# ZHANGKEON/DIS-YOLO

Hardware: AMD Instinct MI355X
Metric: train images/sec @576x576 bf16 (higher is better)
Workload: dtype bf16

## Files before the change

### dis-yolo_amd/csrc/bn.hip

```cpp
#include <stdio.h>
#include <stdlib.h>
#include "common.h"
#include "runtime.h"

namespace {

constexpr int FIN_CPB = 4;
template <int Q>
__device__ __forceinline__ bool block_sum_partials(const float* part, int rows, int C, double* res , int* c_out) {
  constexpr int LANES = 256 / FIN_CPB;
  __shared__ double sh[LANES][FIN_CPB][Q];
  const int cl = threadIdx.x % FIN_CPB, g = threadIdx.x / FIN_CPB;
  const int c = blockIdx.x * FIN_CPB + cl;
  double acc[Q];
#pragma unroll
  for (int q = 0; q < Q; ++q) acc[q] = 0.0;
  if (c < C) {
    int r = g;
    for (; r + 3 * LANES < rows; r += 4 * LANES) {
      float v[4][Q];
#pragma unroll
      for (int u = 0; u < 4; ++u)
#pragma unroll
        for (int q = 0; q < Q; ++q) v[u][q] = part[((size_t)(r + u * LANES) * C + c) * Q + q];
// ... 372 lines not shown
  return ((size_t)colreduce_blocks(rows, C) * C * 2 + 2 * (size_t)C) * sizeof(float);
}

extern "C" int disyolo_bn_act_bwd(const void* dy, const void* x, const float* scale, const float* shift,
                                  const float* mean, const float* rstd, void* dx, float* dgamma, float* dbeta,
                                  int64_t rows, int C, float alpha, void* shortcut_grad, int shortcut_accumulate,
                                  void* workspace, size_t workspace_bytes, void* stream) {
  DY_REQUIRE(dy && x && scale && shift && mean && rstd && dx && dgamma && dbeta, "bn_act_bwd: null pointer");
  DY_REQUIRE(rows > 0 && C > 0 && C % 8 == 0, "bn_act_bwd: bad shape");
  if (workspace_bytes < disyolo_bn_act_bwd_workspace(rows, C) || !workspace) {
    disyolo_set_error("bn_act_bwd: workspace too small");
    return DISYOLO_E_WORKSPACE;
  }
  DY_RECORD_OR_RUN([=](void* s) { return disyolo_bn_act_bwd(dy, x, scale, shift, mean, rstd, dx, dgamma, dbeta, rows, C, alpha, shortcut_grad, shortcut_accumulate, workspace, workspace_bytes, s); });
  hipStream_t s = (hipStream_t)stream;
  const int nb = colreduce_blocks(rows, C), rpb = colreduce_rpb(rows, C);
  const int chunks = C / 8, cpb = chunks < 256 ? chunks : 256;
  float* part = (float*)workspace;
  float* c1 = part + (size_t)nb * C * 2;
  float* c2 = c1 + C;
  hipLaunchKernelGGL(colreduce_kernel<1>, dim3(nb, ceil_div(chunks, cpb)), dim3(256), 0, s, (const uint4*)dy,
                     (const uint4*)x, scale, shift, mean, rstd, alpha, rows, C, rpb, part);
  DY_CHECK_LAUNCH();
  hipLaunchKernelGGL(bn_bwd_finalize_kernel, dim3(ceil_div(C, FIN_CPB)), dim3(256), 0, s, part, nb, C, 1.0 / (double)rows,
                     scale, mean, rstd, dgamma, dbeta, c1, c2);
  DY_CHECK_LAUNCH();
  const int64_t nvec = rows * C / 8;
  hipLaunchKernelGGL(bn_bwd_apply_kernel, dim3(grid_for(nvec)), dim3(256), 0, s, (const uint4*)dy, (const uint4*)x,
                     scale, shift, c1, c2, (uint4*)dx, nvec, C, alpha, (uint4*)shortcut_grad, shortcut_accumulate);
  DY_CHECK_LAUNCH();
  return DISYOLO_OK;
}

extern "C" size_t disyolo_bn_act_bwd_partials_workspace(int C) { return C > 0 ? 2 * (size_t)C * sizeof(float) : 0; }

extern "C" int disyolo_bn_act_bwd_partials(const void* dy, const void* x, const float* scale, const float* shift,
                                           const float* mean, const float* rstd, void* dx, float* dgamma, float* dbeta,
                                           int64_t rows, int C, float alpha, const float* partials, int part_rows,
                                           void* shortcut_grad, int shortcut_accumulate, void* workspace,
                                           size_t workspace_bytes, void* stream) {
  DY_REQUIRE(dy && x && scale && shift && mean && rstd && dx && dgamma && dbeta && partials, "bn_act_bwd_partials: null pointer");
  DY_REQUIRE(rows > 0 && C > 0 && C % 8 == 0 && part_rows > 0, "bn_act_bwd_partials: bad shape");
  if (workspace_bytes < disyolo_bn_act_bwd_partials_workspace(C) || !workspace) {
    disyolo_set_error("bn_act_bwd_partials: workspace too small");
    return DISYOLO_E_WORKSPACE;
  }
  DY_RECORD_OR_RUN([=](void* s) {
    return disyolo_bn_act_bwd_partials(dy, x, scale, shift, mean, rstd, dx, dgamma, dbeta, rows, C, alpha, partials, part_rows,
                                       shortcut_grad, shortcut_accumulate, workspace, workspace_bytes, s);
  });
  hipStream_t s = (hipStream_t)stream;
  float* c1 = (float*)workspace;
  float* c2 = c1 + C;
  hipLaunchKernelGGL(bn_bwd_finalize_kernel, dim3(ceil_div(C, FIN_CPB)), dim3(256), 0, s, partials, part_rows, C,
                     1.0 / (double)rows, scale, mean, rstd, dgamma, dbeta, c1, c2);
  DY_CHECK_LAUNCH();
  const int64_t nvec = rows * C / 8;
  hipLaunchKernelGGL(bn_bwd_apply_kernel, dim3(grid_for(nvec)), dim3(256), 0, s, (const uint4*)dy, (const uint4*)x,
                     scale, shift, c1, c2, (uint4*)dx, nvec, C, alpha, (uint4*)shortcut_grad, shortcut_accumulate);
  DY_CHECK_LAUNCH();
  return DISYOLO_OK;
}

extern "C" int disyolo_bn_partial_sums(const float* partials, int rows, int C, double* sums, void* stream) {
  DY_REQUIRE(partials && sums && rows > 0 && C > 0, "bn_partial_sums: bad args");
  DY_RECORD_OR_RUN([=](void* s) { return disyolo_bn_partial_sums(partials, rows, C, sums, s); });
// ... 122 lines not shown
```

### dis-yolo_amd/lib.py

```python
from __future__ import annotations

import ctypes as C
import os
from typing import Optional

import numpy as np
import torch

_HERE = os.path.dirname(os.path.abspath(__file__))
LIB_PATH = os.environ.get("DISYOLO_LIB", os.path.join(_HERE, "libdisyolo_hip.so"))

GRAD_LD = 32
ROI_MAX = 16
ROI_W = 12
K_MAPS = (3, 5, 7)
MASK_STRIDES = (1, 2, 4)


def roi_w(k: int) -> int:
    return 2 * (k + 1) + 4


def block32_post(k: int) -> int:
    return {3: 1, 5: 2, 7: 3}[k]
# ... 58 lines not shown
    "disyolo_conv_first_fwd_fp8": (C.c_int, [C.c_void_p] * 5 + [C.c_float] + [C.c_int] * 4 + [C.c_float, C.c_void_p]),
    "disyolo_quant_fp8": (C.c_int, [C.c_void_p, C.c_int, C.c_void_p, C.c_int64, C.c_float, C.c_void_p]),
    "disyolo_dequant_fp8": (C.c_int, [C.c_void_p, C.c_void_p, C.c_int64, C.c_float, C.c_void_p]),
    "disyolo_pack_weights_fp8": (C.c_int, [C.c_void_p, C.c_void_p] + [C.c_int] * 3 + [C.c_float, C.c_void_p]),
    "disyolo_conv2d_wgrad_plan": (C.c_int, [C.POINTER(ConvDesc), C.c_int] + [C.POINTER(C.c_int)] * 4),
    "disyolo_conv_first_wgrad_workspace": (C.c_size_t, [C.c_int] * 4),
    "disyolo_conv_first_wgrad": (C.c_int, [C.c_void_p] * 3 + [C.c_int] * 4 + [C.c_void_p, C.c_size_t, C.c_void_p]),
    "disyolo_image_pad8": (C.c_int, [C.c_void_p, C.c_void_p, C.c_int64, C.c_void_p]),
    "disyolo_copy2d_f32": (C.c_int, [C.c_void_p, C.c_void_p] + [C.c_int] * 4 + [C.c_void_p]),
    "disyolo_pack_weights": (C.c_int, [C.c_void_p] * 3 + [C.c_int] * 4 + [C.c_void_p]),
    "disyolo_pack_table_bytes": (C.c_size_t, [C.c_int]),
    "disyolo_pack_table_build": (C.c_int, [C.c_void_p, C.c_int, C.c_void_p, C.POINTER(C.c_int)]),
    "disyolo_pack_all": (C.c_int, [C.c_void_p, C.c_int, C.c_int, C.c_void_p]),
    "disyolo_bn_finalize": (C.c_int, [C.c_void_p, C.c_int, C.c_int, C.c_int64] + [C.c_void_p] * 4 +
                            [C.c_float, C.c_float] + [C.c_void_p] * 5),
    "disyolo_colstats_rows": (C.c_int, [C.c_int64, C.c_int]),
    "disyolo_colstats": (C.c_int, [C.c_void_p, C.c_void_p, C.c_int64, C.c_int, C.c_void_p]),
    "disyolo_bn_fold": (C.c_int, [C.c_void_p] * 4 + [C.c_float] + [C.c_void_p] * 2 + [C.c_int, C.c_void_p]),
    "disyolo_bn_act_fwd": (C.c_int, [C.c_void_p] * 5 + [C.c_int64, C.c_int, C.c_float, C.c_void_p]),
    "disyolo_bn_act_bwd_workspace": (C.c_size_t, [C.c_int64, C.c_int]),
    "disyolo_bn_act_bwd_partials_workspace": (C.c_size_t, [C.c_int]),
    "disyolo_bn_act_bwd_partials": (C.c_int, [C.c_void_p] * 9 + [C.c_int64, C.c_int, C.c_float, C.c_void_p, C.c_int,
                                              C.c_void_p, C.c_int, C.c_void_p, C.c_size_t, C.c_void_p]),
    "disyolo_bn_partial_sums": (C.c_int, [C.c_void_p, C.c_int, C.c_int, C.c_void_p, C.c_void_p]),
    "disyolo_bn_finalize_sums": (C.c_int, [C.c_void_p, C.c_int, C.c_int64] + [C.c_void_p] * 4 + [C.c_float, C.c_float] +
                                 [C.c_void_p] * 5),
    "disyolo_bn_bwd_reduce_rows": (C.c_int, [C.c_int64, C.c_int]),
    "disyolo_bn_bwd_reduce": (C.c_int, [C.c_void_p] * 6 + [C.c_int64, C.c_int, C.c_float, C.c_void_p, C.c_void_p, C.c_size_t,
                                        C.c_void_p]),
    "disyolo_bn_bwd_apply_sums": (C.c_int, [C.c_void_p] * 8 + [C.c_int64] + [C.c_void_p] * 3 + [C.c_int64, C.c_int, C.c_float,
                                            C.c_void_p, C.c_int, C.c_void_p, C.c_size_t, C.c_void_p]),
    "disyolo_bn_act_bwd": (C.c_int, [C.c_void_p] * 9 + [C.c_int64, C.c_int, C.c_float, C.c_void_p, C.c_int, C.c_void_p, C.c_size_t,
                                                       C.c_void_p]),
    "disyolo_upsample2x_bwd": (C.c_int, [C.c_void_p] * 2 + [C.c_int] * 7 + [C.c_void_p]),
    "disyolo_colsum_workspace": (C.c_size_t, [C.c_int64, C.c_int]),
    "disyolo_colsum": (C.c_int, [C.c_void_p, C.c_void_p, C.c_int64, C.c_int, C.c_int, C.c_void_p, C.c_size_t,
                                 C.c_void_p]),
    "disyolo_detect_workspace": (C.c_size_t, [C.c_int] * 3),
    "disyolo_detect": (C.c_int, [C.c_void_p] * 3 + [C.c_int] * 3 + [C.c_void_p] * 2 + [C.c_float, C.c_float, C.c_int] +
                       [C.c_void_p] * 3 + [C.c_size_t, C.c_void_p]),
    "disyolo_yolo_loss_workspace": (C.c_size_t, [C.c_int] * 3),
    "disyolo_yolo_loss": (C.c_int, [C.c_void_p, C.c_void_p, C.c_void_p] + [C.c_int] * 4 + [C.c_void_p, C.c_float] +
                          [C.c_void_p] * 4 + [C.c_size_t, C.c_void_p]),
    "disyolo_shuffle_perm": (C.c_int, [C.c_void_p, C.c_int, C.c_void_p, C.c_int, C.c_int, C.c_uint32, C.c_void_p, C.c_void_p]),
    "disyolo_mask_rois": (C.c_int, [C.c_void_p, C.c_int, C.c_void_p, C.c_int, C.c_void_p, C.c_void_p] + [C.c_int] * 4 +
                          [C.c_float, C.c_void_p, C.c_void_p, C.c_void_p]),
    "disyolo_mask_rois_k": (C.c_int, [C.c_void_p, C.c_int, C.c_void_p, C.c_int, C.c_void_p, C.c_void_p] + [C.c_int] * 5 +
                            [C.c_float, C.c_void_p, C.c_void_p, C.c_void_p]),
    "disyolo_psroi_loss_workspace": (C.c_size_t, [C.c_int, C.c_int]),
    "disyolo_psroi_loss": (C.c_int, [C.c_void_p, C.c_void_p, C.c_int, C.c_void_p, C.c_void_p] + [C.c_int] * 3 +
                           [C.c_float] + [C.c_void_p] * 3 + [C.c_size_t, C.c_void_p]),
    "disyolo_psroi_loss_s": (C.c_int, [C.c_void_p, C.c_void_p, C.c_int, C.c_void_p, C.c_void_p] + [C.c_int] * 4 +
                             [C.c_float] + [C.c_void_p] * 3 + [C.c_size_t, C.c_void_p]),
    "disyolo_psroi_assemble": (C.c_int, [C.c_void_p, C.c_void_p] + [C.c_int] * 4 + [C.c_void_p] * 3),
    "disyolo_mask_paste": (C.c_int, [C.c_void_p, C.c_int, C.c_int, C.c_void_p, C.c_void_p, C.c_int, C.c_int, C.c_void_p,
                                     C.c_void_p, C.c_void_p]),
    "disyolo_letterbox": (C.c_int, [C.c_void_p, C.c_int, C.c_int, C.c_void_p, C.c_int, C.c_void_p, C.c_void_p]),
    "disyolo_confusion16": (C.c_int, [C.c_void_p, C.c_void_p, C.c_int64, C.c_void_p, C.c_void_p]),
    "disyolo_paste_job_size": (C.c_size_t, []),
    "disyolo_paste_job_plan": (C.c_int, [C.c_void_p, C.c_int]),
    "disyolo_mask_paste_iou_batch": (C.c_int, [C.c_void_p, C.c_void_p, C.c_int, C.c_int, C.c_void_p, C.c_void_p]),
    "disyolo_adam_step": (C.c_int, [C.c_void_p] * 4 + [C.c_int64, C.c_int64] + [C.c_float] * 5 + [C.c_int64, C.c_float,
                                                                                             C.c_void_p]),
    "disyolo_adam_step_dev": (C.c_int, [C.c_void_p] * 4 + [C.c_int64, C.c_int64] + [C.c_float] * 5 + [C.c_void_p, C.c_float,
                                                                                                 C.c_void_p]),
    "disyolo_adam_fused_workspace": (C.c_size_t, [C.c_int64]),
# ... 637 lines not shown
    buf = ws.get(load().disyolo_bn_bwd_reduce_rows(rows, C_) * C_ * 2 * 4)
    _check(load().disyolo_bn_bwd_reduce(_p(dy), _p(x), _p(scale), _p(shift), _p(mean), _p(rstd), rows, C_, alpha, _p(sums),
                                        _p(buf), buf.numel(), _stream()), "bn_bwd_reduce")


def bn_bwd_apply_sums(dy, x, scale, shift, mean, rstd, local_sums, global_sums, count, dx, dgamma, dbeta, rows, C_,
                      ws: Workspace, alpha=0.1, shortcut_grad=None, shortcut_accumulate=False) -> None:
    buf = ws.get(2 * C_ * 4)
    _check(load().disyolo_bn_bwd_apply_sums(_p(dy), _p(x), _p(scale), _p(shift), _p(mean), _p(rstd), _p(local_sums),
                                            _p(global_sums), count, _p(dx), _p(dgamma), _p(dbeta), rows, C_, alpha,
                                            _p(shortcut_grad), int(shortcut_accumulate), _p(buf), buf.numel(), _stream()),
           "bn_bwd_apply_sums")


def bn_fold(gamma, beta, mm, mv, eps, scale, shift) -> None:
    _check(load().disyolo_bn_fold(_p(gamma), _p(beta), _p(mm), _p(mv), eps, _p(scale), _p(shift), gamma.numel(),
                                  _stream()), "bn_fold")


def bn_act_fwd(x, scale, shift, residual, y, rows, C_, alpha=0.1) -> None:
    _check(load().disyolo_bn_act_fwd(_p(x), _p(scale), _p(shift), _p(residual), _p(y), rows, C_, alpha, _stream()),
           "bn_act_fwd")


def bn_act_bwd(dy, x, scale, shift, mean, rstd, dx, dgamma, dbeta, rows, C_, ws: Workspace, alpha=0.1,
               shortcut_grad=None, shortcut_accumulate=False) -> None:
    need = load().disyolo_bn_act_bwd_workspace(rows, C_)
    buf = ws.get(need)
    _check(load().disyolo_bn_act_bwd(_p(dy), _p(x), _p(scale), _p(shift), _p(mean), _p(rstd), _p(dx), _p(dgamma),
                                     _p(dbeta), rows, C_, alpha, _p(shortcut_grad), int(shortcut_accumulate), _p(buf),
                                     buf.numel(), _stream()), "bn_act_bwd")


def mask_paste(masks, rects, classids, image_h: int, image_w: int, full_masks, merged) -> None:
    n = int(rects.shape[0])
    if n:
        _need(masks, torch.float32, "masks")
        _need(rects, torch.int32, "rects")
        _need(classids, torch.int32, "classids")
    _check(load().disyolo_mask_paste(_p(masks) if n else None, n, int(masks.shape[-1]) if n else 1, _p(rects) if n else None,
                                     _p(classids) if n else None, image_h, image_w, _p(full_masks), _p(merged), _stream()),
           "mask_paste")


PASTE_JOB = np.dtype([("masks", np.uint64), ("rects", np.uint64), ("classids", np.uint64), ("gt", np.uint64), ("gt_class", np.uint64),
                      ("merged", np.uint64), ("true_map", np.uint64), ("counts", np.uint64), ("n", np.int32), ("ng", np.int32),
                      ("image_h", np.int32), ("image_w", np.int32), ("block0", np.int32), ("reserved", np.int32)])
assert PASTE_JOB.itemsize == 88


def paste_job_plan(jobs) -> int:
    if jobs.dtype != PASTE_JOB or not jobs.flags["C_CONTIGUOUS"] or jobs.ndim != 1:
        raise DisyoloError("paste_job_plan: jobs must be a contiguous 1-d array of PASTE_JOB records")
    rc = load().disyolo_paste_job_plan(jobs.ctypes.data, int(jobs.shape[0]))
    if rc < 0:
        _check(rc, "paste_job_plan")
    return rc


def mask_paste_iou_batch(jobs, jobs_dev, size: int, conf=None) -> None:
    if jobs.dtype != PASTE_JOB or not jobs.flags["C_CONTIGUOUS"] or jobs.ndim != 1:
        raise DisyoloError("mask_paste_iou_batch: jobs must be a contiguous 1-d array of PASTE_JOB records")
    _need(jobs_dev, torch.uint8, "jobs_dev")
    if jobs_dev.numel() < jobs.nbytes:
        raise DisyoloError("mask_paste_iou_batch: %d jobs do not fit %d bytes" % (jobs.shape[0], jobs_dev.numel()))
    if conf is not None:
# ... 308 lines not shown
```

### dis-yolo_amd/net.py

```python
from __future__ import annotations

from typing import Dict, List, Optional, Sequence, Tuple

import math
import json
import contextlib
import os
import sys
import numpy as np
import torch

from . import config as cfg
from . import lib as L

BF16 = torch.bfloat16
F32 = torch.float32

WGRAD_GROUP = 3
OPT_CHUNK_ELEMS = 8_000_000
PIPE_LANE = 2


class Layer:
    __slots__ = ("idx", "cin", "cout", "k", "stride", "kind", "src", "src_up", "shortcut", "lock", "H", "W", "Ho",
                 "Wo", "w", "bias", "gamma", "beta", "mm", "mv", "scale", "shift", "mean", "rstd", "wp", "wdg", "raw",
                 "act", "stats", "stats_rows", "desc", "grad", "grad_set", "need_grad", "dw", "dbias", "dgamma",
                 "dbeta", "dx", "pad_t", "pad_l", "dgrad_descs", "wgrad_desc", "cout_pad",
                 "act8", "w8", "s_w", "s_out", "escale", "desc8", "dual16", "bn_sums", "bwd_local", "bwd_global", "bwd_part", "bwd_part_rows", "wq",
                 "csync", "fused_fwd", "csync_bwd", "fused_bwd")

    def __init__(self, idx, cin, cout, k, stride, kind, src, src_up=None, shortcut=None):
        self.idx, self.cin, self.cout, self.k, self.stride, self.kind = idx, cin, cout, k, stride, kind
        self.src, self.src_up, self.shortcut = src, src_up, shortcut
        for s in self.__slots__[9:]:
            setattr(self, s, None)


MASK_STRIDES = (4, 2, 1)


def build_topology(num_class: int, k_map: int, mask_stride: int = 2) -> List[Layer]:
    if mask_stride not in MASK_STRIDES:
        raise ValueError("mask_stride must be one of %s (got %r)" % (", ".join(map(str, MASK_STRIDES)), mask_stride))
    out_depth = (num_class + 5) * 3
    Ls: List[Layer] = []

    def add(idx, cin, cout, k, s, kind, src, src_up=None, shortcut=None):
        Ls.append(Layer(idx, cin, cout, k, s, kind, src, src_up, shortcut))

    add(1, 3, 32, 3, 1, "bn", 0)
    add(2, 32, 64, 3, 2, "bn", 1)
    i = 3
    ch = 64
    for nblocks, down in ((1, 5), (2, 10), (8, 27), (8, 44), (4, None)):
        for _ in range(nblocks):
            add(i, ch, ch // 2, 1, 1, "bn", i - 1)
            add(i + 1, ch // 2, ch, 3, 1, "res", i, shortcut=i - 1)
            i += 2
        if down:
            add(down, ch, ch * 2, 3, 2, "bn", down - 1)
            ch *= 2
            i = down + 1
# ... 88 lines not shown
        self.plan_only = bool(plan_only)
        if device is None:
            if self.plan_only:
                device = torch.device("cpu")
            elif not torch.cuda.is_available():
                raise L.DisyoloError("YOLONet needs a GPU: the HIP kernels have no CPU fallback")
            else:
                device = torch.device("cuda", torch.cuda.current_device())
        self.device = torch.device(device)
        if not self.plan_only:
            L.load()
            self.ws = L.Workspace(self.device)
            self.ws_aux = L.Workspace(self.device)
            self.ws_det = L.Workspace(self.device)
        self._reg_fresh = False
        self.lock = dict(lock) if lock is not None else {i: (stage == 1 and i <= 52) for i in range(1, self.score_layer + 1)}
        self.layers = build_topology(self.num_class, self.k, self.mask_stride)
        self.by_idx = {l.idx: l for l in self.layers}
        self._lr = float(cfg.LEARNING_RATE)
        self.lr_dev = None
        self.dp = None
        self.sync_bn = False
        self._rec = None
        self._prog = None
        self._prog_marks = []
        self._graph = None
        self.opt_chunks = None
        self._overlap = False
        self._overlap_rec = False
        self._tail_open = False
        self._progs = None
        self.fuse_first_two = True
        self.fuse_blocks = True
        self.use_side_lane = os.environ.get("DISYOLO_SIDE_LANE", "1") != "0"
        self.bn_inkernel = os.environ.get("DISYOLO_BN_INKERNEL", "1") != "0"
        self.bn_inkernel_bwd = os.environ.get("DISYOLO_BN_INKERNEL_BWD", "0") == "1"
        self.bn_fuse_check = None
        self.tail_on_main = 0
        self.pair = bool(backbone_pair)
        self._half = 0
        self._pair_P = 0
        self._init_params(seed, xavier_locked)
        if self.pair:
            if not self.training or self.dtype != "bf16" or self.plan_only:
                raise L.DisyoloError("backbone_pair needs a bf16 training net")
            self._pair_P = self._backbone_prefix()
            if self._pair_P < 2:
                raise L.DisyoloError("backbone_pair needs a locked layer prefix (stage 1)")
        if not self.plan_only:
            self._plan(self.batchsize, self.image_size)

    def _init_params(self, seed: int, xavier_locked: bool) -> None:
        dev = self.device
        g = torch.Generator().manual_seed(seed)
        n_decay = 0
        n_nodecay = 0
        for l in self.layers:
            l.lock = self.lock[l.idx]
            if not l.lock:
                n_decay += l.k * l.k * l.cin * l.cout + (l.cout if l.kind == "lin" else 0)
                if l.kind != "lin":
                    n_nodecay += 2 * l.cout
        self.n_decay, self.n_params = n_decay, n_decay + n_nodecay
        n = max(self.n_params, 1)
        self.arena = torch.zeros(n, dtype=F32, device=dev)
        self.grad_arena = torch.zeros(n, dtype=F32, device=dev)
# ... 922 lines not shown
            if tgt.csync_bwd is None:
                tgt.csync_bwd = L.cluster_sync_buffer(tgt.cout, self.device)
            d = L.make_conv_desc(dx, desc_kw["w"], tgt.dx, k, 1, in_div=in_div, pads=desc_kw["pads"], out_hw=desc_kw["out_hw"],
                                 residual=res, tile=tile_f,
                                 bn_bwd=(tgt.raw, tgt.scale, tgt.shift, tgt.mean, tgt.rstd, tgt.bwd_part, cfg.ALPHA),
                                 bn_bwd_fused=dict(dgamma=tgt.dgamma, dbeta=tgt.dbeta, sync=tgt.csync_bwd))
            tgt.fused_bwd = True
        L.conv2d_fwd(d)

    def check_cluster_sync(self) -> None:
        for l in self.layers:
            for name, buf in (("forward", l.csync), ("backward", l.csync_bwd)):
                if buf is not None:
                    code = L.cluster_sync_error(buf, l.cout)
                    if code:
                        raise L.DisyoloError("conv%d: the in-launch batch-norm exchange (%s) timed out (code %#x): another launch of "
                                             "that kind was running on this device, or the grid was not resident; the results of "
                                             "this run are wrong (DISYOLO_BN_INKERNEL=0 switches the feature off)" % (l.idx, name, code))

    def _shortcut_feeds_grad(self, tgt: Layer) -> bool:
        return tgt.shortcut is not None and self.by_idx[tgt.shortcut].grad is not None

    def _final_writers(self, visit) -> Dict[int, Tuple[int, str]]:
        last: Dict[int, Tuple[int, str]] = {}
        for l in visit:
            if l.lock:
                continue
            if l.kind != "lin" and l.shortcut is not None and self.by_idx[l.shortcut].grad is not None:
                last[l.shortcut] = (l.idx, "add")
            for mode, tgt, _ in l.dgrad_descs:
                last[tgt.idx] = (l.idx, mode)
        return last

    def backward_order(self) -> List[Layer]:
        heads = [self.by_idx[i] for i in (75, 74, 67, 66, 59, 58)]
        return heads + [l for l in reversed(self.layers) if l.idx not in self.HEAD_LAYERS]

    def backward(self, on_layer_done=None, sweep: bool = False) -> None:
        B = self.B
        for l in self.layers:
            l.grad_set = False
        visit = self.backward_order()
        order = [l for l in visit if not l.lock]
        final_of = {} if self.sync_bn else self._final_writers(visit)
        for l in self.layers:
            l.bwd_part_rows = 0
            l.fused_bwd = False
        inl = self.dp is not None and self.dp.inlist
        overlap_opt = sweep and (self.dp is None or inl) and self.n_params > 0
        if overlap_opt:
            if self.opt_chunks is None:
                self._plan_opt_chunks()
            self._opt_swept = set()
            self._opt_done = [set() for _ in self.opt_chunks]
        pending: list = []

        def flush():
            if not pending:
                return
            side_g = pending[0][4]
            mark = L.lane_mark(0) if side_g else None
            waited = False
            for (pl, pdx, pld, pM, pside) in pending:
                if pside:
                    if not waited:
                        L.lane_wait(mark, 1)
                        waited = True
                    L.set_lane(1)
                wsl = self.ws_aux if pside else self.ws
                if pl.kind == "lin":
                    L.colsum(pl.dx, pl.dbias, pM, pl.cout_pad, pl.cout, wsl)
                if pl.idx == 1:
                    L.conv_first_wgrad(self.images, pl.dx, pl.dw, wsl)
                else:
                    L.conv2d_wgrad(pl.wgrad_desc, pdx, pld, pl.dw, wsl)
                if pside:
                    L.set_lane(0)
                if self._overlap_rec:
                    for src, reader in self._xstep_reader.items():
                        if reader == pl.idx and self._xstep_slot[src] in self._xstep_waits.values():
                            L.lane_mark_slot(1 if pside else 0, self._xstep_slot[src])
                if overlap_opt and pside:
                    ci = self._opt_chunk_of[pl.idx]
                    self._opt_done[ci].add(pl.idx)
                    if self._opt_done[ci] == self.opt_chunks[ci]["members"]:
                        if inl:
                            L.lane_wait(L.lane_mark(1), L.COMM_LANE)
                            L.set_lane(L.COMM_LANE)
                            ch = self.opt_chunks[ci]
                            self.dp.exchange_inlist(ci, ch["off"], ch["cnt"])
                            self._sweep_chunk(ci, 1.0 / self.dp.world_size)
                            L.set_lane(0)
                        else:
                            L.set_lane(1)
                            self._sweep_chunk(ci, 1.0)
                            L.set_lane(0)
                if on_layer_done is not None:
                    on_layer_done(pl)
            pending.clear()

        for l in visit:
            pos = order.index(l) if not l.lock else -1
            if l.idx == self.score_layer and getattr(self, "_mask_loss_pending", False):
                L.lane_wait(self._mask_mark, 0)
                self._mask_loss_pending = False
            if l.lock:
                continue
            M = B * l.Ho * l.Wo
            if l.kind == "lin":
                dx, ld = l.dx, l.cout_pad
            else:
                if not l.grad_set:
                    raise L.DisyoloError("layer %d received no gradient" % l.idx)
                sc = self.by_idx[l.shortcut] if l.shortcut is not None else None
                if sc is not None and sc.grad is None:
                    sc = None
                kw = dict(shortcut_grad=sc.grad, shortcut_accumulate=sc.grad_set) if sc is not None else {}
                if l.fused_bwd:
                    pass
                elif self.sync_bn:
                    L.bn_bwd_reduce(l.grad, l.raw, l.scale, l.shift, l.mean, l.rstd, M, l.cout, l.bwd_local, self.ws, cfg.ALPHA)
                    L.copy2d_f32(l.bwd_local.view(torch.float32), l.bwd_global.view(torch.float32), 1, 4 * l.cout,
                                 4 * l.cout, 4 * l.cout)
                    self._sync_sums(l.bwd_global)
                    L.bn_bwd_apply_sums(l.grad, l.raw, l.scale, l.shift, l.mean, l.rstd, l.bwd_local, l.bwd_global,
                                        M * self.dp.world_size, l.dx, l.dgamma, l.dbeta, M, l.cout, self.ws, cfg.ALPHA, **kw)
                elif l.bwd_part_rows:
                    ref = None
                    if self.bn_fuse_check is not None and self._rec is None:
                        ref = (torch.empty_like(l.dx), torch.empty_like(l.dgamma), torch.empty_like(l.dbeta))
                        L.bn_act_bwd(l.grad, l.raw, l.scale, l.shift, l.mean, l.rstd, ref[0], ref[1], ref[2], M, l.cout,
                                     self.ws, cfg.ALPHA)
                    L.bn_act_bwd_partials(l.grad, l.raw, l.scale, l.shift, l.mean, l.rstd, l.dx, l.dgamma, l.dbeta, M,
                                          l.cout, l.bwd_part, l.bwd_part_rows, self.ws, cfg.ALPHA, **kw)
                    if ref is not None:
                        torch.cuda.synchronize()

                        def rel(a, b):
                            a, b = a.double().flatten(), b.double().flatten()
                            return float((a - b).norm() / (b.norm() + 1e-30))
                        self.bn_fuse_check.append({"layer": l.idx, "rows": l.bwd_part_rows, "shape": (l.Ho, l.Wo, l.cout),
                                                   "dx": rel(l.dx, ref[0]), "dgamma": rel(l.dgamma, ref[1]),
                                                   "dbeta": rel(l.dbeta, ref[2]),
                                                   "finite": bool(torch.isfinite(l.dx.float()).all())})
                else:
                    L.bn_act_bwd(l.grad, l.raw, l.scale, l.shift, l.mean, l.rstd, l.dx, l.dgamma, l.dbeta, M, l.cout,
                                 self.ws, cfg.ALPHA, **kw)
                dx, ld = l.dx, l.cout
                if sc is not None:
                    sc.grad_set = True
            tail = self.tail_on_main if (self.dp is None or inl) else 0
            side = self.use_side_lane and (pos < len(order) - tail)
            for mode, tgt, kw in l.dgrad_descs:
                if mode == "direct":
                    final = (final_of.get(tgt.idx) == (l.idx, "direct") and not tgt.lock and tgt.kind != "lin"
                             and tgt.cout % 8 == 0 and tgt.raw is not None)
                    self._accumulate_into(tgt, kw, dx, l.cin, l.k, l.stride, final)
                    tgt.grad_set = True
                else:
                    self._accumulate_into(tgt, kw, dx, l.cin, l.k, l.stride)
                    up = tgt
                    L.upsample2x_bwd(kw["tmp"], up.grad, B, l.H, l.W, up.cout, 0, up.cout, accumulate=up.grad_set)
                    up.grad_set = True
            if pending and pending[-1][4] != side:
                flush()
            pending.append((l, dx, ld, M, side))
            if not side or len(pending) >= WGRAD_GROUP:
                flush()
        flush()
        if not self._overlap_rec:
            L.lane_sync(1, 0)

    def _apply_tiles(self) -> None:
        for l in self.layers:
            if l.stats is not None and l.idx > 1:
                l.stats = None
        self._build_descs()
        if self.training:
            self._build_dgrad_descs()

    def autotune(self, reps: int = 3, candidates=None, det_thresh: float = cfg.OBJ_THRESHOLD, cache=None) -> dict:
        if self._prog is not None:
            raise L.DisyoloError("autotune() must run before build_program()")
        if cache and os.path.exists(cache):
            with open(cache) as f:
                picks = {tuple(json.loads(k)): int(v) for k, v in json.load(f).items()}
            L.TUNED.clear()
            L.TUNED.update({k: v for k, v in picks.items() if v})
            self._apply_tiles()
            self.tuned = picks
            return picks
        state = {k: v.clone() for k, v in self.state_dict().items()} if self.training else None
        saved_stats = {}
        for l in self.layers:
            if l.stats is not None and l.idx > 1:
                saved_stats[l.idx] = (l.stats, l.stats_rows)
                l.stats = torch.zeros(-(-self.B * l.Ho * l.Wo // 64), l.cout, 2, dtype=F32, device=self.device)
        if saved_stats:
            self._build_descs()
        tuner = L.ConvTuner(candidates or L.TUNE_CANDIDATES)
        L.TUNED.clear()
# ... 363 lines not shown
```

### include/disyolo.h

```cpp
#ifndef DISYOLO_H
#define DISYOLO_H

#include <stddef.h>
#include <stdint.h>

#ifdef __cplusplus
extern "C" {
#endif

#define DISYOLO_OK 0
#define DISYOLO_E_ARG (-1)
#define DISYOLO_E_WORKSPACE (-2)
#define DISYOLO_E_HIP (-3)

#define DISYOLO_GRAD_LD 32
#define DISYOLO_ROI_MAX 16
#define DISYOLO_ROI_W 12
#define DISYOLO_ROI_W_K(k) (2 * ((k) + 1) + 4)

int disyolo_version(void);
const char* disyolo_last_error(void);

enum {
  DISYOLO_CONV_LEAKY = 1,
// ... 121 lines not shown
size_t disyolo_pack_table_bytes(int njobs);
int disyolo_pack_table_build(const disyolo_pack_job* jobs, int njobs, void* host_table, int* total_blocks);
int disyolo_pack_all(const void* device_table, int njobs, int total_blocks, void* stream);

int disyolo_bn_finalize(const float* stats, int rows, int C, int64_t count, const float* gamma,
                        const float* beta, float* moving_mean, float* moving_var, float decay,
                        float eps, float* scale, float* shift, float* mean, float* rstd,
                        void* stream);
int disyolo_bn_partial_sums(const float* partials, int rows, int C, double* sums, void* stream);
int disyolo_bn_finalize_sums(const double* sums, int C, int64_t count, const float* gamma, const float* beta,
                             float* moving_mean, float* moving_var, float decay, float eps, float* scale,
                             float* shift, float* mean, float* rstd, void* stream);
int disyolo_bn_bwd_reduce_rows(int64_t rows, int C);
int disyolo_bn_bwd_reduce(const void* dy, const void* x, const float* scale, const float* shift,
                          const float* mean, const float* rstd, int64_t rows, int C, float alpha, double* sums,
                          void* workspace, size_t workspace_bytes, void* stream);
int disyolo_bn_bwd_apply_sums(const void* dy, const void* x, const float* scale, const float* shift,
                              const float* mean, const float* rstd, const double* local_sums,
                              const double* global_sums, int64_t count, void* dx, float* dgamma, float* dbeta,
                              int64_t rows, int C, float alpha, void* shortcut_grad, int shortcut_accumulate,
                              void* workspace, size_t workspace_bytes, void* stream);
int disyolo_colstats_rows(int64_t rows, int C);
int disyolo_colstats(const void* x, float* stats, int64_t rows, int C, void* stream);
int disyolo_bn_fold(const float* gamma, const float* beta, const float* moving_mean,
                    const float* moving_var, float eps, float* scale, float* shift, int C,
                    void* stream);
int disyolo_bn_act_fwd(const void* x, const float* scale, const float* shift, const void* residual,
                       void* y, int64_t rows, int C, float alpha, void* stream);
size_t disyolo_bn_act_bwd_workspace(int64_t rows, int C);
int disyolo_bn_act_bwd(const void* dy, const void* x, const float* scale, const float* shift,
                       const float* mean, const float* rstd, void* dx, float* dgamma, float* dbeta,
                       int64_t rows, int C, float alpha, void* shortcut_grad, int shortcut_accumulate,
                       void* workspace, size_t workspace_bytes, void* stream);
size_t disyolo_bn_act_bwd_partials_workspace(int C);
int disyolo_bn_act_bwd_partials(const void* dy, const void* x, const float* scale, const float* shift,
                                const float* mean, const float* rstd, void* dx, float* dgamma,
                                float* dbeta, int64_t rows, int C, float alpha, const float* partials,
                                int part_rows, void* shortcut_grad, int shortcut_accumulate, void* workspace,
                                size_t workspace_bytes, void* stream);

int disyolo_upsample2x_bwd(const void* src, void* dst, int B, int Hs, int Ws, int src_C, int c_off,
                           int C, int accumulate, void* stream);
size_t disyolo_colsum_workspace(int64_t rows, int C);
int disyolo_colsum(const void* x, float* out, int64_t rows, int C, int out_C, void* workspace,
                   size_t workspace_bytes, void* stream);

size_t disyolo_detect_workspace(int B, int S, int num_class);
int disyolo_detect(const float* logits3, const float* logits2, const float* logits1, int B, int S,
                   int num_class, const float* anchors_host, const float* clip_window,
                   float obj_thresh, float nms_thresh, int max_det, float* detections,
                   int32_t* det_count, void* workspace, size_t workspace_bytes, void* stream);

size_t disyolo_yolo_loss_workspace(int B, int S, int num_class);
int disyolo_yolo_loss(const float* const logits[3], const float* const labels[3],
                      const float* true_boxes, int max_boxes, int B, int S, int num_class,
                      const float* anchors_host, float ignore_thresh, const float scales[4],
                      void* const dlogits[3], float* losses, void* workspace,
                      size_t workspace_bytes, void* stream);

int disyolo_mask_rois_k(const float* detections, int max_det, const float* true_boxes, int G,
                        const int32_t* perm_det, const int32_t* perm_gt, int B, int map_size, int k,
                        int n_det, int n_gt, float iou_thresh, int32_t* rois, int32_t* roi_count,
                        void* stream);
int disyolo_mask_rois(const float* detections, int max_det, const float* true_boxes, int G,
                      const int32_t* perm_det, const int32_t* perm_gt, int B, int map_size,
                      int n_det, int n_gt, float iou_thresh, int32_t* rois, int32_t* roi_count,
// ... 118 lines not shown
```

Before: 2126.

## Fuse 1x1 linear-layer data gradient into the following BN-activation backward

For a 1x1 stride-1 linear layer whose only data-gradient target is the next BN+leaky layer, the gradient is no longer materialized. Instead the BN backward recomputes it on the fly with MFMA from the linear layer's output gradient and weights, once in the sums pass and once in the apply pass. This removes writing and re-reading a large bf16 gradient temporary for big layers (at least 500k rows) and the separate dgrad GEMM launch. In exchange the small GEMM runs twice, weight-gradient enqueue is deferred by one layer, and the path is limited to C up to 128 with no shortcut, no sync BN and no other writers.

```diff
diff --git a/dis-yolo_amd/csrc/bn.hip b/dis-yolo_amd/csrc/bn.hip
--- a/dis-yolo_amd/csrc/bn.hip
+++ b/dis-yolo_amd/csrc/bn.hip
@@ -428,6 +428,14 @@
   return DISYOLO_OK;
 }
 
+int bn_bwd_finalize_launch(const float* part, int rows, int C, double inv_count, const float* scale, const float* mean,
+                           const float* rstd, float* dgamma, float* dbeta, float* cA, float* cC, void* stream) {
+  hipLaunchKernelGGL(bn_bwd_finalize_kernel, dim3(ceil_div(C, FIN_CPB)), dim3(256), 0, (hipStream_t)stream, part, rows, C,
+                     inv_count, scale, mean, rstd, dgamma, dbeta, cA, cC);
+  DY_CHECK_LAUNCH();
+  return DISYOLO_OK;
+}
+
 extern "C" size_t disyolo_bn_act_bwd_partials_workspace(int C) { return C > 0 ? 2 * (size_t)C * sizeof(float) : 0; }
 
 extern "C" int disyolo_bn_act_bwd_partials(const void* dy, const void* x, const float* scale, const float* shift,
diff --git a/dis-yolo_amd/csrc/bn_lin.hip b/dis-yolo_amd/csrc/bn_lin.hip
--- /dev/null
+++ b/dis-yolo_amd/csrc/bn_lin.hip
@@ -0,0 +1,230 @@
+#include <stdio.h>
+#include <stdlib.h>
+#include "common.h"
+#include "runtime.h"
+
+int bn_bwd_finalize_launch(const float* part, int rows, int C, double inv_count, const float* scale, const float* mean,
+                           const float* rstd, float* dgamma, float* dbeta, float* cA, float* cC, void* stream);
+
+namespace {
+
+constexpr int TM = 64;
+
+template <int LD>
+struct LinTile {
+  static constexpr int WROW = LD * 2 + 16;
+  static __device__ __forceinline__ int grow(int C) { return C * 2 + 16; }
+  static __host__ __device__ size_t bytes(int C) { return (size_t)C * WROW + (size_t)TM * (C * 2 + 16); }
+
+  static __device__ __forceinline__ void load_panel(const bf16* wdg, char* sW, int C) {
+    constexpr int CPR = LD / 8;
+    const uint4* src = reinterpret_cast<const uint4*>(wdg);
+    for (int v = threadIdx.x; v < C * CPR; v += 256) {
+      const int n = v / CPR, c = v - n * CPR;
+      *reinterpret_cast<uint4*>(sW + n * WROW + c * 16) = src[v];
+    }
+  }
+
+  static __device__ __forceinline__ void grad_tile(const bf16* dy, int64_t t0, int64_t row_end, const char* sW, char* sG,
+                                                   int C) {
+    constexpr int KK = LD / 32;
+    const int lane = threadIdx.x & 63, wave = threadIdx.x >> 6;
+    const int frow = lane & 15, fchunk = lane >> 4;
+    const int64_t m = t0 + wave * 16 + frow;
+    bf16x8 xf[KK];
+#pragma unroll
+    for (int kk = 0; kk < KK; ++kk) {
+      uint4 u = make_uint4(0u, 0u, 0u, 0u);
+      if (m < row_end) u = *reinterpret_cast<const uint4*>(dy + m * LD + (kk * 4 + fchunk) * 8);
+      xf[kk] = __builtin_bit_cast(bf16x8, u);
+    }
+    const int GROW = grow(C);
+    const int nj = C >> 4;
+    for (int j = 0; j < nj; ++j) {
+      f32x4 acc = f32x4{0.f, 0.f, 0.f, 0.f};
+#pragma unroll
+      for (int kk = 0; kk < KK; ++kk) {
+        const bf16x8 wf = *reinterpret_cast<const bf16x8*>(sW + (j * 16 + frow) * WROW + (kk * 4 + fchunk) * 16);
+        acc = __builtin_amdgcn_mfma_f32_16x16x32_bf16(wf, xf[kk], acc, 0, 0, 0);
+      }
+      float v[4];
+#pragma unroll
+      for (int r = 0; r < 4; ++r) v[r] = acc[r] * 1.f + 0.f;
+      uint2 o2;
+      o2.x = pack2(v[0], v[1]);
+      o2.y = pack2(v[2], v[3]);
+      *reinterpret_cast<uint2*>(sG + (wave * 16 + frow) * GROW + (j * 16 + fchunk * 4) * 2) = o2;
+    }
+  }
+};
+
+template <int LD>
+__global__ __launch_bounds__(256) void bn_lin_sums_kernel(const bf16* dy, const bf16* wdg, const uint4* b, const float* scale,
+                                                          const float* shift, const float* mean, const float* rstd,
+                                                          float alpha, int64_t rows, int C, int rows_per_block, float* part) {
+  using LT = LinTile<LD>;
+  extern __shared__ __attribute__((aligned(16))) char smem[];
+  char* sW = smem;
+  char* sG = smem + C * LT::WROW;
+  float* sh = reinterpret_cast<float*>(smem);
+  const int GROW = LT::grow(C);
+  const int chunks = C / 8;
+  const int cpb = chunks;
+  const int lanes = 256 / cpb;
+  const int cl = threadIdx.x % cpb, rl = threadIdx.x / cpb;
+  const int chunk = cl;
+  const int c0 = chunk * 8;
+  float acc[16];
+#pragma unroll
+  for (int k = 0; k < 16; ++k) acc[k] = 0.f;
+  const bool active = rl < lanes;
+  LT::load_panel(wdg, sW, C);
+  float sc[8], shf[8], mu[8], rs[8];
+#pragma unroll
+  for (int k = 0; k < 8; ++k) {
+    sc[k] = scale[c0 + k];
+    shf[k] = shift[c0 + k];
+    mu[k] = mean[c0 + k];
+    rs[k] = rstd[c0 + k];
+  }
+  const int64_t r0 = (int64_t)blockIdx.x * rows_per_block;
+  int64_t r1 = r0 + rows_per_block;
+  if (r1 > rows) r1 = rows;
+  for (int64_t t0 = r0; t0 < r1; t0 += TM) {
+    __syncthreads();
+    LT::grad_tile(dy, t0, r1, sW, sG, C);
+    __syncthreads();
+    if (active) {
+      const int off = (int)((t0 - r0) % lanes);
+      int lr = rl - off;
+      if (lr < 0) lr += lanes;
+      for (; lr < TM && t0 + lr < r1; lr += lanes) {
+        const int64_t r = t0 + lr;
+        float va[8];
+        unpack8(*reinterpret_cast<const uint4*>(sG + lr * GROW + chunk * 16), va);
+        float vx[8];
+        unpack8(b[r * chunks + chunk], vx);
+#pragma unroll
+        for (int k = 0; k < 8; ++k) {
+          const float z = vx[k] * sc[k] + shf[k];
+          const float g = va[k] * (z > 0.f ? 1.f : alpha);
+          const float xh = (vx[k] - mu[k]) * rs[k];
+          acc[k] += g;
+          acc[8 + k] += g * xh;
+        }
+      }
+    }
+  }
+  __syncthreads();
+#pragma unroll
+  for (int k = 0; k < 16; ++k) sh[threadIdx.x * 16 + k] = acc[k];
+  __syncthreads();
+  if (rl == 0) {
+    for (int l = 1; l < lanes; ++l) {
+#pragma unroll
+      for (int k = 0; k < 16; ++k) acc[k] += sh[(l * cpb + cl) * 16 + k];
+    }
+#pragma unroll
+    for (int k = 0; k < 8; ++k) {
+#pragma unroll
+      for (int q = 0; q < 2; ++q) part[((size_t)blockIdx.x * C + c0 + k) * 2 + q] = acc[q * 8 + k];
+    }
+  }
+}
+
+__device__ __forceinline__ void lin_load8(const float* p, float* o) {
+  const float4 a = *reinterpret_cast<const float4*>(p), c = *reinterpret_cast<const float4*>(p + 4);
+  o[0] = a.x; o[1] = a.y; o[2] = a.z; o[3] = a.w; o[4] = c.x; o[5] = c.y; o[6] = c.z; o[7] = c.w;
+}
+
+template <int LD>
+__global__ __launch_bounds__(256) void bn_lin_apply_kernel(const bf16* dy, const bf16* wdg, const uint4* x, const float* scale,
+                                                           const float* shift, const float* cA, const float* cC, uint4* dx,
+                                                           int64_t rows, int C, float alpha) {
+  using LT = LinTile<LD>;
+  extern __shared__ __attribute__((aligned(16))) char smem[];
+  char* sW = smem;
+  char* sG = smem + C * LT::WROW;
+  const int GROW = LT::grow(C);
+  const int chunks = C >> 3;
+  LT::load_panel(wdg, sW, C);
+  const int64_t ntiles = (rows + TM - 1) / TM;
+  for (int64_t tile = blockIdx.x; tile < ntiles; tile += gridDim.x) {
+    const int64_t t0 = tile * TM;
+    __syncthreads();
+    LT::grad_tile(dy, t0, rows, sW, sG, C);
+    __syncthreads();
+    for (int v = threadIdx.x; v < TM * chunks; v += 256) {
+      const int lr = v / chunks, ch = v - lr * chunks;
+      const int64_t r = t0 + lr;
+      if (r >= rows) break;
+      const int c0 = ch << 3;
+      const int64_t i = r * chunks + ch;
+      float g[8], vx[8], sc[8], sh[8], A[8], Cc[8];
+      unpack8(*reinterpret_cast<const uint4*>(sG + lr * GROW + ch * 16), g);
+      unpack8(x[i], vx);
+      lin_load8(scale + c0, sc);
+      lin_load8(shift + c0, sh);
+      lin_load8(cA + c0, A);
+      lin_load8(cC + c0, Cc);
+#pragma unroll
+      for (int k = 0; k < 8; ++k) {
+        const float z = vx[k] * sc[k] + sh[k];
+        const float gg = g[k] * (z > 0.f ? 1.f : alpha);
+        g[k] = sc[k] * gg - vx[k] * A[k] + Cc[k];
+      }
+      dx[i] = pack8(g);
+    }
+  }
+}
+
+template <int LD>
+int launch_lin(const bf16* dy, const bf16* wdg, const void* x, const float* scale, const float* shift, const float* mean,
+               const float* rstd, void* dx, float* dgamma, float* dbeta, int64_t rows, int C, float alpha, float* part,
+               hipStream_t s) {
+  const int nb = disyolo_bn_bwd_reduce_rows(rows, C);
+  const int rpb = (int)((rows + nb - 1) / nb);
+  float* c1 = part + (size_t)nb * C * 2;
+  float* c2 = c1 + C;
+  size_t lds = LinTile<LD>::bytes(C);
+  const size_t red = (size_t)256 * 16 * sizeof(float);
+  hipLaunchKernelGGL((bn_lin_sums_kernel<LD>), dim3(nb), dim3(256), lds < red ? red : lds, s, dy, wdg, (const uint4*)x, scale,
+                     shift, mean, rstd, alpha, rows, C, rpb, part);
+  DY_CHECK_LAUNCH();
+  const int rc = bn_bwd_finalize_launch(part, nb, C, 1.0 / (double)rows, scale, mean, rstd, dgamma, dbeta, c1, c2, s);
+  if (rc != DISYOLO_OK) return rc;
+  const int64_t ntiles = (rows + TM - 1) / TM;
+  const int grid = (int)(ntiles < 2048 ? ntiles : 2048);
+  hipLaunchKernelGGL((bn_lin_apply_kernel<LD>), dim3(grid), dim3(256), lds, s, dy, wdg, (const uint4*)x, scale, shift, c1, c2,
+                     (uint4*)dx, rows, C, alpha);
+  DY_CHECK_LAUNCH();
+  return DISYOLO_OK;
+}
+}
+
+extern "C" int disyolo_bn_act_bwd_lin_ok(int64_t rows, int C, int ld, int shortcut_grad, int sync_bn, int other_writers) {
+  if (rows <= 0 || C <= 0 || C % 16 || C > 128) return 0;
+  if (ld != 32 && ld != 64) return 0;
+  if (shortcut_grad || sync_bn || other_writers) return 0;
+  return 1;
+}
+
+extern "C" int disyolo_bn_act_bwd_lin(const void* dy, int ld, const void* wdg, const void* x, const float* scale,
+                                      const float* shift, const float* mean, const float* rstd, void* dx, float* dgamma,
+                                      float* dbeta, int64_t rows, int C, float alpha, void* workspace, size_t workspace_bytes,
+                                      void* stream) {
+  DY_REQUIRE(dy && wdg && x && scale && shift && mean && rstd && dx && dgamma && dbeta, "bn_act_bwd_lin: null pointer");
+  DY_REQUIRE(disyolo_bn_act_bwd_lin_ok(rows, C, ld, 0, 0, 0), "bn_act_bwd_lin: unsupported shape (rows %lld, C %d, ld %d; ask "
+             "disyolo_bn_act_bwd_lin_ok)", (long long)rows, C, ld);
+  if (workspace_bytes < disyolo_bn_act_bwd_workspace(rows, C) || !workspace) {
+    disyolo_set_error("bn_act_bwd_lin: workspace too small");
+    return DISYOLO_E_WORKSPACE;
+  }
+  DY_RECORD_OR_RUN([=](void* s) { return disyolo_bn_act_bwd_lin(dy, ld, wdg, x, scale, shift, mean, rstd, dx, dgamma, dbeta, rows, C, alpha, workspace, workspace_bytes, s); });
+  hipStream_t s = (hipStream_t)stream;
+  if (ld == 32)
+    return launch_lin<32>((const bf16*)dy, (const bf16*)wdg, x, scale, shift, mean, rstd, dx, dgamma, dbeta, rows, C, alpha,
+                          (float*)workspace, s);
+  return launch_lin<64>((const bf16*)dy, (const bf16*)wdg, x, scale, shift, mean, rstd, dx, dgamma, dbeta, rows, C, alpha,
+                        (float*)workspace, s);
+}
diff --git a/dis-yolo_amd/lib.py b/dis-yolo_amd/lib.py
--- a/dis-yolo_amd/lib.py
+++ b/dis-yolo_amd/lib.py
@@ -114,6 +114,9 @@
                                             C.c_void_p, C.c_int, C.c_void_p, C.c_size_t, C.c_void_p]),
     "disyolo_bn_act_bwd": (C.c_int, [C.c_void_p] * 9 + [C.c_int64, C.c_int, C.c_float, C.c_void_p, C.c_int, C.c_void_p, C.c_size_t,
                                                        C.c_void_p]),
+    "disyolo_bn_act_bwd_lin_ok": (C.c_int, [C.c_int64, C.c_int, C.c_int, C.c_int, C.c_int, C.c_int]),
+    "disyolo_bn_act_bwd_lin": (C.c_int, [C.c_void_p, C.c_int] + [C.c_void_p] * 9 + [C.c_int64, C.c_int, C.c_float, C.c_void_p,
+                                                                                  C.c_size_t, C.c_void_p]),
     "disyolo_upsample2x_bwd": (C.c_int, [C.c_void_p] * 2 + [C.c_int] * 7 + [C.c_void_p]),
     "disyolo_colsum_workspace": (C.c_size_t, [C.c_int64, C.c_int]),
     "disyolo_colsum": (C.c_int, [C.c_void_p, C.c_void_p, C.c_int64, C.c_int, C.c_int, C.c_void_p, C.c_size_t,
@@ -817,6 +820,21 @@
                                      buf.numel(), _stream()), "bn_act_bwd")
 
 
+def bn_act_bwd_lin_ok(rows, C_, ld, shortcut_grad=False, sync_bn=False, other_writers=False) -> bool:
+    return load().disyolo_bn_act_bwd_lin_ok(rows, C_, ld, int(shortcut_grad), int(sync_bn), int(other_writers)) == 1
+
+
+def bn_act_bwd_lin(lin_dy, ld, wdg, x, scale, shift, mean, rstd, dx, dgamma, dbeta, rows, C_, ws: Workspace, alpha=0.1) -> None:
+    _need(lin_dy, torch.bfloat16, "lin_dy")
+    _need(wdg, torch.bfloat16, "wdg")
+    if lin_dy.numel() < rows * ld or wdg.numel() < C_ * ld or not wdg.is_contiguous():
+        raise DisyoloError("bn_act_bwd_lin: lin_dy / wdg smaller than rows x ld / C x ld")
+    buf = ws.get(load().disyolo_bn_act_bwd_workspace(rows, C_))
+    _check(load().disyolo_bn_act_bwd_lin(_p(lin_dy), ld, _p(wdg), _p(x), _p(scale), _p(shift), _p(mean), _p(rstd), _p(dx),
+                                         _p(dgamma), _p(dbeta), rows, C_, alpha, _p(buf), buf.numel(), _stream()),
+           "bn_act_bwd_lin")
+
+
 def mask_paste(masks, rects, classids, image_h: int, image_w: int, full_masks, merged) -> None:
     n = int(rects.shape[0])
     if n:
diff --git a/dis-yolo_amd/net.py b/dis-yolo_amd/net.py
--- a/dis-yolo_amd/net.py
+++ b/dis-yolo_amd/net.py
@@ -18,6 +18,7 @@
 
 WGRAD_GROUP = 3
 OPT_CHUNK_ELEMS = 8_000_000
+FUSE_GRAD_MIN_ROWS = 500_000
 PIPE_LANE = 2
 
 
@@ -27,7 +28,7 @@
                  "act", "stats", "stats_rows", "desc", "grad", "grad_set", "need_grad", "dw", "dbias", "dgamma",
                  "dbeta", "dx", "pad_t", "pad_l", "dgrad_descs", "wgrad_desc", "cout_pad",
                  "act8", "w8", "s_w", "s_out", "escale", "desc8", "dual16", "bn_sums", "bwd_local", "bwd_global", "bwd_part", "bwd_part_rows", "wq",
-                 "csync", "fused_fwd", "csync_bwd", "fused_bwd")
+                 "csync", "fused_fwd", "csync_bwd", "fused_bwd", "lin_grad")
 
     def __init__(self, idx, cin, cout, k, stride, kind, src, src_up=None, shortcut=None):
         self.idx, self.cin, self.cout, self.k, self.stride, self.kind = idx, cin, cout, k, stride, kind
@@ -182,6 +183,8 @@
         self._progs = None
         self.fuse_first_two = True
         self.fuse_blocks = True
+        self.fuse_grad_temps = True
+        self.fuse_grad_min_rows = FUSE_GRAD_MIN_ROWS
         self.use_side_lane = os.environ.get("DISYOLO_SIDE_LANE", "1") != "0"
         self.bn_inkernel = os.environ.get("DISYOLO_BN_INKERNEL", "1") != "0"
         self.bn_inkernel_bwd = os.environ.get("DISYOLO_BN_INKERNEL_BWD", "0") == "1"
@@ -1170,6 +1173,33 @@
                 last[tgt.idx] = (l.idx, mode)
         return last
 
+    def _lin_grad_targets(self, visit) -> Dict[int, Layer]:
+        if (not self.fuse_grad_temps or L.TUNER is not None or self.bn_fuse_check is not None or self.sync_bn
+                or self.bn_inkernel_bwd):
+            return {}
+        writers: Dict[int, int] = {}
+        for l in visit:
+            if l.lock:
+                continue
+            if l.kind != "lin" and l.shortcut is not None and self.by_idx[l.shortcut].grad is not None:
+                writers[l.shortcut] = writers.get(l.shortcut, 0) + 1
+            for _, tgt, _ in l.dgrad_descs:
+                writers[tgt.idx] = writers.get(tgt.idx, 0) + 1
+        out: Dict[int, Layer] = {}
+        for l, nxt in zip(visit, visit[1:]):
+            if l.lock or l.kind != "lin" or l.k != 1 or l.stride != 1 or len(l.dgrad_descs) != 1:
+                continue
+            mode, tgt, kw = l.dgrad_descs[0]
+            if mode != "direct" or "quad" in kw or tgt is not nxt or tgt.lock or tgt.kind == "lin" or tgt.raw is None:
+                continue
+            M = self.B * tgt.Ho * tgt.Wo
+            if M >= self.fuse_grad_min_rows and L.bn_act_bwd_lin_ok(M, tgt.cout, l.cout_pad,
+                                                                      shortcut_grad=self._shortcut_feeds_grad(tgt),
+                                                                      sync_bn=self.sync_bn,
+                                                                      other_writers=writers.get(tgt.idx, 0) != 1):
+                out[l.idx] = tgt
+        return out
+
     def backward_order(self) -> List[Layer]:
         heads = [self.by_idx[i] for i in (75, 74, 67, 66, 59, 58)]
         return heads + [l for l in reversed(self.layers) if l.idx not in self.HEAD_LAYERS]
@@ -1181,9 +1211,11 @@
         visit = self.backward_order()
         order = [l for l in visit if not l.lock]
         final_of = {} if self.sync_bn else self._final_writers(visit)
+        lin_tgt = self._lin_grad_targets(visit)
         for l in self.layers:
             l.bwd_part_rows = 0
             l.fused_bwd = False
+            l.lin_grad = None
         inl = self.dp is not None and self.dp.inlist
         overlap_opt = sweep and (self.dp is None or inl) and self.n_params > 0
         if overlap_opt:
@@ -1192,6 +1224,7 @@
             self._opt_swept = set()
             self._opt_done = [set() for _ in self.opt_chunks]
         pending: list = []
+        held: list = []
 
         def flush():
             if not pending:
@@ -1237,6 +1270,13 @@
                     on_layer_done(pl)
             pending.clear()
 
+        def enqueue_wgrad(l, dx, ld, M, side):
+            if pending and pending[-1][4] != side:
+                flush()
+            pending.append((l, dx, ld, M, side))
+            if not side or len(pending) >= WGRAD_GROUP:
+                flush()
+
         for l in visit:
             pos = order.index(l) if not l.lock else -1
             if l.idx == self.score_layer and getattr(self, "_mask_loss_pending", False):
@@ -1256,6 +1296,10 @@
                 kw = dict(shortcut_grad=sc.grad, shortcut_accumulate=sc.grad_set) if sc is not None else {}
                 if l.fused_bwd:
                     pass
+                elif l.lin_grad is not None:
+                    src = l.lin_grad
+                    L.bn_act_bwd_lin(src.dx, src.cout_pad, src.wdg, l.raw, l.scale, l.shift, l.mean, l.rstd, l.dx, l.dgamma,
+                                     l.dbeta, M, l.cout, self.ws, cfg.ALPHA)
                 elif self.sync_bn:
                     L.bn_bwd_reduce(l.grad, l.raw, l.scale, l.shift, l.mean, l.rstd, M, l.cout, l.bwd_local, self.ws, cfg.ALPHA)
                     L.copy2d_f32(l.bwd_local.view(torch.float32), l.bwd_global.view(torch.float32), 1, 4 * l.cout,
@@ -1287,10 +1331,16 @@
                 dx, ld = l.dx, l.cout
                 if sc is not None:
                     sc.grad_set = True
+            for h in held:
+                enqueue_wgrad(*h)
+            held.clear()
             tail = self.tail_on_main if (self.dp is None or inl) else 0
             side = self.use_side_lane and (pos < len(order) - tail)
             for mode, tgt, kw in l.dgrad_descs:
-                if mode == "direct":
+                if mode == "direct" and lin_tgt.get(l.idx) is tgt:
+                    tgt.lin_grad = l
+                    tgt.grad_set = True
+                elif mode == "direct":
                     final = (final_of.get(tgt.idx) == (l.idx, "direct") and not tgt.lock and tgt.kind != "lin"
                              and tgt.cout % 8 == 0 and tgt.raw is not None)
                     self._accumulate_into(tgt, kw, dx, l.cin, l.k, l.stride, final)
@@ -1300,11 +1350,10 @@
                     up = tgt
                     L.upsample2x_bwd(kw["tmp"], up.grad, B, l.H, l.W, up.cout, 0, up.cout, accumulate=up.grad_set)
                     up.grad_set = True
-            if pending and pending[-1][4] != side:
-                flush()
-            pending.append((l, dx, ld, M, side))
-            if not side or len(pending) >= WGRAD_GROUP:
-                flush()
+            if l.idx in lin_tgt:
+                held.append((l, dx, ld, M, side))
+            else:
+                enqueue_wgrad(l, dx, ld, M, side)
         flush()
         if not self._overlap_rec:
             L.lane_sync(1, 0)
diff --git a/include/disyolo.h b/include/disyolo.h
--- a/include/disyolo.h
+++ b/include/disyolo.h
@@ -177,6 +177,11 @@
                        const float* mean, const float* rstd, void* dx, float* dgamma, float* dbeta,
                        int64_t rows, int C, float alpha, void* shortcut_grad, int shortcut_accumulate,
                        void* workspace, size_t workspace_bytes, void* stream);
+int disyolo_bn_act_bwd_lin_ok(int64_t rows, int C, int ld, int shortcut_grad, int sync_bn, int other_writers);
+int disyolo_bn_act_bwd_lin(const void* lin_dy, int ld, const void* wdg, const void* x, const float* scale,
+                           const float* shift, const float* mean, const float* rstd, void* dx, float* dgamma,
+                           float* dbeta, int64_t rows, int C, float alpha, void* workspace, size_t workspace_bytes,
+                           void* stream);
 size_t disyolo_bn_act_bwd_partials_workspace(int C);
 int disyolo_bn_act_bwd_partials(const void* dy, const void* x, const float* scale, const float* shift,
                                 const float* mean, const float* rstd, void* dx, float* dgamma,
```

New measurement: 2143, median of 3. About the same (+0.8%).
